# DrSleep/nas-segm-pytorch

Hardware: AMD Instinct MI355X
Metric: images/sec (fwd+bwd+optimizer step) WACV arch0 2048x1024 bs=4/GPU (higher is better)
Workload: dtype f32

## Files before the change

include/nasseg.h:

```cpp
#ifndef NASSEG_H
#define NASSEG_H

#include <stdint.h>

#ifdef __cplusplus
extern "C" {
#endif

const char* nasseg_last_error(void);
int nasseg_abi_version(void);
int nasseg_device_count(void);

int nasseg_dw_pack_weight(const float* w, float* wt, int C, int K, int flip, void* stream);
int nasseg_dwconv(const float* x, const float* wt, float* y, const float* in_scale,
                  const float* in_shift, int in_act, const float* scale, const float* shift, int act,
                  int B, int H, int W, int C, int Ho, int Wo, int K, int stride, int pad, int dil,
                  int transposed, float* stats, void* stream);
int nasseg_dwconv_strip_ok(int K, int stride, int dil);
int64_t nasseg_dwconv_stats_blocks(int B, int C, int Ho, int Wo, int K, int stride, int dil);
int nasseg_dwconv_bwd_data_bn(const float* dy, const float* wt, float* g, const float* z,
                              const float* scale, const float* shift, const float* mean,
                              const float* invstd, int act, int B, int H, int W, int C, int Ho,
                              int Wo, int K, int stride, int pad, int dil, int transposed,
                              float* stats, void* stream);
// ... 35 lines not shown
                    int in_act, const float* bn1_scale, const float* bn1_shift, const float* bn1_mean,
                    const float* bn1_invstd, int act1, const float* bn2_scale, const float* bn2_shift,
                    const float* bn2_mean, const float* bn2_invstd, const float* bn2_sums, int bn2_train, int bn2_act,
                    int B, int H, int W, int K, int C, int Ho, int Wo, int stride, float* stats, void* stream);

int nasseg_conv_pack_weight(const float* w, float* wp, int N, int K, int kh, int kw, int mode,
                            void* stream);
int nasseg_pack_weights(int count, const float* const* w, float* const* wp, const int* dims,
                        void* stream);
int nasseg_conv_fwd_pack_mode(int K, int kh, int kw);
int nasseg_conv_fwd(const float* x, int ldx, const float* wp, float* y, int ldy,
                    const float* in_scale, const float* in_shift, int in_act,
                    const float* out_scale, const float* out_shift, int out_act, const float* res,
                    int ldres, int B, int Hs, int Ws, int K, int Ho, int Wo, int N, int kh, int kw,
                    int stride, int pad, int dil, int transposed, float* stats, void* stream);
int64_t nasseg_conv_fwd_stats_blocks(int B, int Ho, int Wo, int N, int K, int pointwise);
int64_t nasseg_conv_fwd_stats_rows(int B, int Ho, int Wo, int N, int K, int kh, int kw, int stride, int pad, int dil);
int64_t nasseg_conv_pw_min_pixels(int64_t v);
int nasseg_conv_pwn_mode(int v);
int nasseg_conv_deep_k(int v);
int nasseg_pool_strip(int v);
int64_t nasseg_conv_pointwise_kernel(int B, int Ho, int Wo, int N, int K, int pointwise);
int64_t nasseg_conv_fwd_lds3x3(int B, int Ho, int Wo, int N, int K, int kh, int kw, int stride, int pad, int dil,
                               int with_stats);
int nasseg_conv_bwd_data_bn(const float* dy, int lddy, const float* wp, float* g, int ldg,
                            const float* z, int ldz, const float* scale, const float* shift,
                            const float* mean, const float* invstd, int act, int B, int Hs, int Ws,
                            int K, int Ho, int Wo, int N, int kh, int kw, int stride, int pad,
                            int dil, float* stats, void* stream);
int nasseg_conv_wgrad_lds3x3(int B, int Hs, int Ws, int K, int Ho, int Wo, int N, int kh, int kw, int stride,
// ... 16 lines not shown
int nasseg_dwconv_wgrad_bn(const float* x, const float* g, const float* z, float* dz, float* dw, float* ws,
                           const float* in_scale, const float* in_shift, int in_act, const float* bn_scale, const float* bn_shift,
                           const float* bn_mean, const float* bn_invstd, const float* bn_sums, int bn_train, int bn_act,
                           int B, int H, int W, int C, int Ho, int Wo, int K, int stride, int pad, int dil,
                           void* stream);
int64_t nasseg_conv_pw_bwd_slabs(int B, int H, int W, int K, int N);
int64_t nasseg_conv_pw_bwd_reads_z(int B, int H, int W, int K, int N);
int64_t nasseg_conv_pw_bwd_kernel_id(int B, int H, int W, int K, int N, int z_null);
int64_t nasseg_conv_pw_bwd_rz_min_pixels(int64_t v);
int nasseg_conv_pw_bwd_bn(const float* x, const float* g, const float* z, const float* wb, float* dx, float* dw,
                          float* ws, const float* in_scale, const float* in_shift, int in_act, int dx_act,
                          const float* bn_scale, const float* bn_shift, const float* bn_mean, const float* bn_invstd,
                          const float* bn_sums, int bn_train, int bn_act, int B, int H, int W, int K, int N,
                          const float* in_mean, const float* in_invstd, float* dx_stats, const float* dx_res,
                          void* stream);
int nasseg_conv_wgrad(const float* x, int ldx, const float* dy, int lddy, float* dw, float* ws,
                      const float* in_scale, const float* in_shift, int in_act, int B, int Hs,
                      int Ws, int K, int Ho, int Wo, int N, int kh, int kw, int stride, int pad,
                      int dil, void* stream);

int64_t nasseg_colred_workspace(int S, int64_t R, int C);
int nasseg_colred(int mode, const float* a, int64_t lda, const float* b, int64_t ldb,
                  const float* c, int64_t ldc, float* out, float* ws, int S, int64_t R, int C,
                  float mul, void* stream);
int nasseg_bn_stats(const float* x, int64_t ldx, int64_t M, int C, float eps, float momentum,
                    const float* gamma, const float* beta, float* mean, float* invstd,
                    float* scale, float* shift, float* running_mean, float* running_var,
                    int64_t* num_batches_tracked, float* ws, void* stream);
int nasseg_bn_finalize(float* partial, int nblk, int64_t M, int C, float eps, float momentum,
                       const float* gamma, const float* beta, float* mean, float* invstd,
// ... 294 lines not shown
                         const float* bn2_scale, const float* bn2_shift, const float* bn2_mean,
                         const float* bn2_invstd, const float* bn2_sums, int bn2_train, int bn2_act, int B, int H, int W,
                         int K, int C, int Ho, int Wo, int stride, float* stats, void* stream);
int nasseg_bf16_dwconv_bwd_bn(const nasseg_bf16_t* xz, const nasseg_bf16_t* g, const nasseg_bf16_t* z, const float* wt,
                              int wt_flipped, nasseg_bf16_t* ge, float* dw, float* ws, const float* in_scale, const float* in_shift,
                              const float* in_mean, const float* in_invstd, int in_act, const float* bn_scale,
                              const float* bn_shift, const float* bn_mean, const float* bn_invstd, const float* bn_sums,
                              int bn_train, int bn_act, int B, int H, int W, int C, int Ho, int Wo, int K, int stride,
                              int pad, int dil, float* stats, void* stream);
int nasseg_bf16_conv_pw_bwd_bn(const nasseg_bf16_t* x, const nasseg_bf16_t* g, const nasseg_bf16_t* z, const float* wb,
                               nasseg_bf16_t* dx, float* dw, float* ws, const float* in_scale, const float* in_shift,
                               int in_act, int dx_act, const float* bn_scale, const float* bn_shift, const float* bn_mean,
                               const float* bn_invstd, const float* bn_sums, int bn_train, int bn_act, int B, int H,
                               int W, int K, int N, const float* in_mean, const float* in_invstd, float* dx_stats,
                               const nasseg_bf16_t* dx_res, void* stream);
int nasseg_bf16_sepconv_fwd(const nasseg_bf16_t* x, const float* wdw, const float* wpw, nasseg_bf16_t* zdw,
                            nasseg_bf16_t* y, const float* in_scale, const float* in_shift, int in_act,
                            const float* out_scale, const float* out_shift, int out_act, int B, int H, int W, int C,
                            int Ho, int Wo, int N, int K, int stride, int pad, int dil, float* stats, void* stream);
int nasseg_bf16_affine_act(const nasseg_bf16_t* x, const float* scale, const float* shift, const nasseg_bf16_t* res,
                      nasseg_bf16_t* y, int64_t n, int C, int act, void* stream);
int nasseg_bf16_psum_bwd(const nasseg_bf16_t* dy, const nasseg_bf16_t* za, const float* tsa, int act_a, const float* ca,
                         nasseg_bf16_t* ga, float* part_a, const nasseg_bf16_t* zb, const float* tsb, int act_b,
                         const float* cb, nasseg_bf16_t* gb, float* part_b, float* cpart, int B, int H, int W, int C,
                         void* stream);
int nasseg_bf16_add_act2(const nasseg_bf16_t* xa, const float* sa, const float* ha, int act_a, const float* ca,
                         const nasseg_bf16_t* xb, const float* sb, const float* hb, int act_b, const float* cb,
                         nasseg_bf16_t* y, int64_t n, int C, void* stream);
int nasseg_bf16_bn_bwd_apply(const nasseg_bf16_t* dy, const nasseg_bf16_t* x, const float* scale, const float* shift,
                        const float* mean, const float* invstd, const float* sums, int64_t M,
// ... 178 lines not shown
                  int B, int H, int W, int C, int Ho, int Wo, int K, int stride, int pad, int dil,
                  int transposed, float* stats, void* stream);
int nasseg_bf16_dwconv_bwd_data_bn(const nasseg_bf16_t* dy, const float* wt, nasseg_bf16_t* g, const nasseg_bf16_t* z,
                              const float* scale, const float* shift, const float* mean,
                              const float* invstd, int act, int B, int H, int W, int C, int Ho,
                              int Wo, int K, int stride, int pad, int dil, int transposed,
                              float* stats, void* stream);
int nasseg_bf16_dwconv_wgrad(const nasseg_bf16_t* x, const nasseg_bf16_t* dy, float* dw, float* ws,
                        const float* in_scale, const float* in_shift, int in_act, int B, int H, int W,
                        int C, int Ho, int Wo, int K, int stride, int pad, int dil, void* stream);
int nasseg_bf16_conv_fwd(const nasseg_bf16_t* x, int ldx, const float* wp, nasseg_bf16_t* y, int ldy,
                    const float* in_scale, const float* in_shift, int in_act,
                    const float* out_scale, const float* out_shift, int out_act, const nasseg_bf16_t* res,
                    int ldres, int B, int Hs, int Ws, int K, int Ho, int Wo, int N, int kh, int kw,
                    int stride, int pad, int dil, int transposed, float* stats, void* stream);
int nasseg_bf16_conv_bwd_data_bn(const nasseg_bf16_t* dy, int lddy, const float* wp, nasseg_bf16_t* g, int ldg,
                            const nasseg_bf16_t* z, int ldz, const float* scale, const float* shift,
                            const float* mean, const float* invstd, int act, int B, int Hs, int Ws,
                            int K, int Ho, int Wo, int N, int kh, int kw, int stride, int pad,
                            int dil, float* stats, void* stream);
int nasseg_bf16_conv_wgrad_many(int count, const int64_t* desc, void* stream);
int nasseg_bf16_dwconv_wgrad_many(int count, const int64_t* desc, void* stream);
int nasseg_bf16_conv_wgrad_bn(const nasseg_bf16_t* x, int ldx, const nasseg_bf16_t* g, int ldg,
                              const nasseg_bf16_t* z, int ldz, nasseg_bf16_t* dz, int lddz, float* dw, float* ws,
                              const float* in_scale, const float* in_shift, int in_act, const float* bn_scale, const float* bn_shift,
                              const float* bn_mean, const float* bn_invstd, const float* bn_sums, int bn_train, int bn_act,
                              int B, int H, int W, int K, int N, void* stream);
int nasseg_bf16_conv_wgrad_bn_flat(const nasseg_bf16_t* x, int ldx, const nasseg_bf16_t* g, int ldg,
                                   const nasseg_bf16_t* z, int ldz, float* dw, float* ws, const float* bn_scale,
                                   const float* bn_shift, const float* bn_mean, const float* bn_invstd,
// ... 40 lines not shown
```

nas-segm-pytorch_amd/csrc/conv_fwd.hip:

```cpp
#include "conv_args.h"

#include <atomic>
#include <cstdio>
#include <cstdlib>

#if NASSEG_FP32_ONLY
std::atomic<int> g_conv_deep_k{1};
#else
extern std::atomic<int> g_conv_deep_k;
#endif

namespace {

enum { KM_VEC = 0, KM_SCALAR = 1, KM_FLAT = 2 };

#ifndef NASSEG_CONV_KU
#define NASSEG_CONV_KU 1
#endif
#ifndef NASSEG_PW_MIN_PIXELS
#define NASSEG_PW_MIN_PIXELS -2
#endif
#ifndef NASSEG_LDS3X3_VALU_TAIL
#define NASSEG_LDS3X3_VALU_TAIL 1
#endif
// ... 348 lines not shown
  p.nt = pw_round_tiles(cdiv(N, 16));
  if (!p.nt) return p;
  p.mt = p.nt <= 6 ? 2 : 1;
  const int KP = (K + 15) & ~15;
  p.lds = ((size_t)p.nt * 16 * (KP + 4) + 2 * KP + 4 * 2 * p.nt * 16) * sizeof(float);
  if (p.lds > (size_t)(64 << 10)) return p;
  int r = p.nt <= 2 ? 4 : (p.nt <= 4 ? 3 : (p.nt == 9 ? 3 : 2));
  const int by_lds = (int)((size_t)(160 << 10) / p.lds);
  if (r > by_lds) r = by_lds;
  const int64_t wg_tiles = cdiv64(cdiv64(M, 16 * p.mt), 4);
  p.grid = (int)(wg_tiles < 256LL * r ? wg_tiles : 256LL * r);
  p.ok = 1;
  return p;
}

template <int NT, int MT, int STATS>
__global__ __launch_bounds__(256) void conv_pw_kernel(FwdArgs a) {
  constexpr bool kSums = STATS == 1 || STATS == 2;
  constexpr int NPc = NT * 16;
  extern __shared__ float smem[];
  const int K = a.K, N = a.N;
  const int KP = (K + 15) & ~15, LSK = KP + 4, nkb = KP >> 4;
  float* wl = smem;
  float* psc = wl + NPc * LSK;
  float* psh = psc + KP;
  float* sred = psh + KP;
  const int tid = threadIdx.x;
  const int lane = tid & 63, wave = tid >> 6;
  const int j = lane & 15, kg = lane >> 4;
  const int Mtot = a.g.B * a.g.Ho * a.g.Wo;
  const int ntiles = (Mtot + 16 * MT - 1) / (16 * MT);

  for (int it = tid; it < NPc * (KP >> 2); it += 256) {
    const int n = it / (KP >> 2), k = (it - n * (KP >> 2)) * 4;
    const float4 v = keep_if(lda4(a.w + (int64_t)(n < N ? n : 0) * K + (k < K ? k : 0)), n < N && k < K);
    *reinterpret_cast<float4*>(&wl[n * LSK + k]) = v;
  }
  const bool pro = a.in_scale || a.in_shift || a.in_act;
  for (int k = tid; k < KP; k += 256) {
    psc[k] = (a.in_scale && k < K) ? a.in_scale[k] : 1.f;
    psh[k] = (a.in_shift && k < K) ? a.in_shift[k] : 0.f;
  }
  for (int t = tid; t < 4 * 2 * NPc; t += 256) sred[t] = 0.f;
  __syncthreads();
  const ActSel pact = act_sel(a.in_act);
  float* my_red = sred + wave * 2 * NPc;

  f32x4 acc[MT][NT];
#pragma unroll
  for (int mt = 0; mt < MT; ++mt)
#pragma unroll
    for (int nt = 0; nt < NT; ++nt) acc[mt][nt] = (f32x4){0.f, 0.f, 0.f, 0.f};

  const int wstride = gridDim.x * 4;
  int tl = blockIdx.x * 4 + wave, kl = 0;
  float4 ring[kPwD][MT];
  auto load_step = [&](float4* dst) {
    const int tc = tl < ntiles ? tl : ntiles - 1;
    const int k = kl * 16 + kg * 4;
#pragma unroll
    for (int mt = 0; mt < MT; ++mt) {
      const int m = tc * (16 * MT) + mt * 16 + j;
      dst[mt] = lda4(a.x + (int64_t)(m < Mtot ? m : Mtot - 1) * a.ldx + (k < K ? k : 0));
    }
    if (++kl == nkb) {
      kl = 0;
      tl += wstride;
    }
  };
#pragma unroll
  for (int d = 0; d < kPwD; ++d) load_step(ring[d]);

  int tc = blockIdx.x * 4 + wave, kc = 0;
  bool more = tc < ntiles;
  while (more) {
#pragma unroll
    for (int d = 0; d < kPwD; ++d) {
      if (tc >= ntiles) {
// ... 117 lines not shown
        for (int mt = 0; mt < MT; ++mt) acc[mt][nt] = (f32x4){0.f, 0.f, 0.f, 0.f};
        if ((nt & 1) == 1) __builtin_amdgcn_sched_barrier(0);
      }
    }
  }
  if (kSums) {
    __syncthreads();
    for (int t = tid; t < NPc; t += 256) {
      if (t < N) {
        float* po = a.stats + (int64_t)blockIdx.x * 2 * N + t;
        po[0] = (sred[t] + sred[2 * NPc + t]) + (sred[4 * NPc + t] + sred[6 * NPc + t]);
        po[N] = (sred[NPc + t] + sred[3 * NPc + t]) + (sred[5 * NPc + t] + sred[7 * NPc + t]);
      }
    }
  }
}

__global__ void conv_pack_kernel(const float* __restrict__ w, float* __restrict__ wp, int N, int K,
                                 int ntaps, int mode) {
  const int64_t i = (int64_t)blockIdx.x * blockDim.x + threadIdx.x;
  const int64_t total = (int64_t)ntaps * N * K;
  if (i >= total) return;
  int tap, n, k;
  if (mode == 0) {
    k = (int)(i % K);
    int64_t t = i / K;
    n = (int)(t % N);
    tap = (int)(t / N);
  } else if (mode == 1) {
    n = (int)(i % N);
// ... 565 lines not shown
  return NASSEG_OK;
}
int launch_pw(const FwdArgs& a, const PwFwdPlan& p, int stats, hipStream_t s) {
  switch (p.nt) {
    case 1: return launch_pw_nt<1, 2>(a, p, stats, s);
    case 2: return launch_pw_nt<2, 2>(a, p, stats, s);
    case 3: return launch_pw_nt<3, 2>(a, p, stats, s);
    case 4: return launch_pw_nt<4, 2>(a, p, stats, s);
    case 6: return launch_pw_nt<6, 2>(a, p, stats, s);
    case 9: return launch_pw_nt<9, 1>(a, p, stats, s);
    case 12: return launch_pw_nt<12, 1>(a, p, stats, s);
    default: return launch_pw_nt<14, 1>(a, p, stats, s);
  }
}

inline bool conv_small_ws(int64_t Mtot, int N, int K) {
  return g_conv_deep_k.load() != 0 && Mtot <= kDeepKMaxPixels && (N & 3) == 0 && (K & 3) == 0 && K >= 8 &&
         (int64_t)N * K <= 196608;
}

inline bool lds3x3_geometry(int B, int Ho, int Wo, int N, int K, int kh, int kw, int stride, int pad, int dil) {
  return kh == 3 && kw == 3 && stride == 1 && dil >= 1 && dil <= kLdsMaxDil && K * 9 > 64 && cdiv(N, 16) <= 4 &&
         Wo >= kLdsTW && Ho >= kLdsTH && B <= 65535 && pad >= 0 && pad <= 2 * dil;
}

inline int fwd_pack_mode(int K, int kh, int kw) { return (kh * kw > 1 && kh * kw * K <= 64) ? 2 : 0; }

int conv_dispatch(FwdArgs& a, int stats_mode, hipStream_t s) {
  const int K = a.K, N = a.N;
  const ConvGeom& g = a.g;
// ... 185 lines not shown
                    const float* in_scale, const float* in_shift, int in_act,
                    const float* out_scale, const float* out_shift, int out_act, const act_t* res,
                    int ldres, int B, int Hs, int Ws, int K, int Ho, int Wo, int N, int kh, int kw,
                    int stride, int pad, int dil, int transposed, float* stats, void* stream) {
  FwdArgs a = {};
  a.x = x; a.ldx = ldx; a.w = wp; a.y = y; a.ldy = ldy;
  a.in_scale = in_scale; a.in_shift = in_shift; a.in_act = in_act;
  a.out_scale = out_scale; a.out_shift = out_shift; a.out_act = out_act;
  a.res = res; a.ldres = ldres; a.stats = stats; a.K = K; a.N = N;
  a.g.B = B; a.g.Hs = Hs; a.g.Ws = Ws; a.g.Ho = Ho; a.g.Wo = Wo;
  a.g.kh = kh; a.g.kw = kw; a.g.stride = stride; a.g.pad = pad; a.g.dil = dil;
  a.g.transposed = transposed;
  return conv_dispatch(a, stats ? 1 : 0, (hipStream_t)stream);
}

int NASSEG_FN(conv_bwd_data_bn)(const act_t* dy, int lddy, const float* wp, act_t* g, int ldg,
                            const act_t* z, int ldz, const float* scale, const float* shift,
                            const float* mean, const float* invstd, int act, int B, int Hs, int Ws,
                            int K, int Ho, int Wo, int N, int kh, int kw, int stride, int pad,
                            int dil, float* stats, void* stream) {
  NASSEG_REQUIRE(z && (!stats || (scale && shift && mean && invstd)), "conv_bwd_data_bn: null argument");
  NASSEG_REQUIRE((ldz & 3) == 0 && ldz >= N, "conv_bwd_data_bn: bad ldz");
  FwdArgs a = {};
  a.x = dy; a.ldx = lddy; a.w = wp; a.y = g; a.ldy = ldg;
  a.stats = stats; a.K = K; a.N = N;
  a.bz = z; a.ldbz = ldz; a.b_scale = scale; a.b_shift = shift; a.b_mean = mean;
  a.b_invstd = invstd; a.b_act = act;
  a.g.B = B; a.g.Hs = Hs; a.g.Ws = Ws; a.g.Ho = Ho; a.g.Wo = Wo;
  a.g.kh = kh; a.g.kw = kw; a.g.stride = stride; a.g.pad = pad; a.g.dil = dil;
  a.g.transposed = 1;
// ... 5 lines not shown
```

nas-segm-pytorch_amd/csrc/conv_pwbwd.hip:

```cpp
#include <atomic>
#include <cstdlib>
#include <type_traits>

#include "conv_common.h"

#if NASSEG_FP32_ONLY
std::atomic<int64_t> g_pw_rz_min_pixels{1 << 18};
#else
extern std::atomic<int64_t> g_pw_rz_min_pixels;
#endif

namespace {

#ifndef NASSEG_PW_CHUNK
#define NASSEG_PW_CHUNK 3
#endif
#ifndef NASSEG_PW_RECOMPUTE_Z
#define NASSEG_PW_RECOMPUTE_Z 1
#endif
constexpr int kPwTile = 64;
constexpr int kPwMaxTiles = 24;

struct PwArgs {
  const act_t* x;
// ... 343 lines not shown
      __syncthreads();
      if (wave == 0) {
#pragma unroll
        for (int r = 0; r < 4; ++r) {
          const float v = acc2[nt][kt][r] + red[(0 * 64 + lane) * 4 + r] + red[(1 * 64 + lane) * 4 + r] +
                          red[(2 * 64 + lane) * 4 + r];
          const int n = nt * 16 + 4 * kg + r, k = kt * 16 + j;
          if (n < N && k < K) pout[(int64_t)n * K + k] = v;
        }
      }
    }
}

constexpr int kPwChunk = 64;
constexpr int kW2LS = kPwChunk + 4;
template <int KC, bool PRO>
__global__ __launch_bounds__(256, 2) void conv_pw_bwd_wide_kernel(PwArgs a) {
  extern __shared__ float smem[];
  constexpr int LS = kW2LS;
  float* dzt = smem;
  float* xt = dzt + kPwTile * LS;
  float* wt = xt + kPwTile * LS;
  float* wt0 = wt + kPwChunk * LS;
  float* ca = wt0 + kPwChunk * LS;
  float* cb = ca + 64;
  float* cd = cb + 64;
  float* cs = cd + 64;
  float* psc = cs + 64;
  float* psh = psc + KC * kPwChunk;
  const int tid = threadIdx.x;
  const int lane = tid & 63, wave = tid >> 6;
  const int j = lane & 15, kg = lane >> 4;
  const int N = a.N, K = a.K;
  for (int n = tid; n < 64; n += 256) {
    float va = 0.f, vb = 0.f, vd = 0.f, vs = 0.f;
    if (n < N) {
      const float sc = a.bn_scale[n];
      va = sc;
      vs = a.bn_act ? a.bn_shift[n] : 0.f;
      if (a.bn_train) {
        const float is = a.bn_invstd[n], mu = a.bn_mean[n];
        const float s0 = a.bn_sums[n] * a.invM, s1 = a.bn_sums[N + n] * a.invM;
        vb = -sc * is * s1;
        vd = sc * (mu * is * s1 - s0);
      }
    }
    ca[n] = va; cb[n] = vb; cd[n] = vd; cs[n] = vs;
  }
// ... 15 lines not shown
  const float m_lo = a.bn_act ? 0.f : -__builtin_inff();
  const float m_hi = a.bn_act == NASSEG_ACT_RELU6 ? 6.f : __builtin_inff();
  const int irow = tid >> 4, icol = (tid & 15) * 4;
  float4 XN[4], WN[4], GN[4], ZN[4];
  auto issue_gz = [&](int t0) {
#pragma unroll
    for (int u = 0; u < 4; ++u) {
      const int p = t0 + irow + 16 * u;
      const int64_t off = (int64_t)(p < p_end ? p : p_end - 1) * N + (icol < N ? icol : 0);
      GN[u] = lda4(a.g + off);
      ZN[u] = lda4(a.z + off);
    }
  };
  auto issue_xw = [&](int t0, int kc) {
    const int k = kc + icol;
#pragma unroll
    for (int u = 0; u < 4; ++u) {
      const int p = t0 + irow + 16 * u;
      XN[u] = lda4(a.x + (int64_t)(p < p_end ? p : p_end - 1) * K + (k < K ? k : 0));
      if (kc) {
        const int kw = kc + irow + 16 * u;
        WN[u] = ld4(a.wb + (int64_t)(kw < K ? kw : 0) * N + (icol < N ? icol : 0));
      }
    }
  };
  auto place_gz = [&](int t0) {
    const float4 va = ld4(ca + icol), vb = ld4(cb + icol), vd = ld4(cd + icol), vs = ld4(cs + icol);
#pragma unroll
    for (int u = 0; u < 4; ++u) {
      const int px = irow + 16 * u;
      const bool ok = t0 + px < p_end && icol < N;
      float4 gv = GN[u];
      const float4 zv = ZN[u];
      {
// ... 70 lines not shown
              const int n = ns * 16 + kg * 4;
              const float4 bv = *reinterpret_cast<const float4*>(brow + n);
              float4 av[NQ];
#pragma unroll
              for (int q = 0; q < NQ; ++q) av[q] = *reinterpret_cast<const float4*>(&wcur[(q * 16 + j) * LS + n]);
#pragma unroll
              for (int q = 0; q < NQ; ++q) acc1[q] = mfma16(av[q].x, bv.x, acc1[q]);
#pragma unroll
              for (int q = 0; q < NQ; ++q) acc1[q] = mfma16(av[q].y, bv.y, acc1[q]);
#pragma unroll
              for (int q = 0; q < NQ; ++q) acc1[q] = mfma16(av[q].z, bv.z, acc1[q]);
#pragma unroll
              for (int q = 0; q < NQ; ++q) acc1[q] = mfma16(av[q].w, bv.w, acc1[q]);
            }
            const bool pok = p < p_end;
            act_t* prow = a.dx + (int64_t)(pok ? p : p_begin) * K + kc + kg * 4;
#pragma unroll
            for (int q = 0; q < NQ; ++q) {
              const int kl = q * 16 + kg * 4;
              float4 o = make_float4(acc1[q][0], acc1[q][1], acc1[q][2], acc1[q][3]);
              if (a.dx_act)
                o = mul4(o, act_mask_of(*reinterpret_cast<const float4*>(&xt[(wave * 16 + j) * LS + kl]), a.dx_act));
              if (pok && kc + kl < K) sta4(prow + q * 16, a.dx_res ? add4(o, rres[q]) : o);
            }
          }
          if (own) {
            auto dw_chunk = [&](f32x4 (&acc)[4]) {
#pragma unroll 2
              for (int u = 0; u < kPwTile / 4; ++u) {
                const int pl = u * 4 + kg;
                const float av = dzt[pl * LS + wave * 16 + j];
// ... 21 lines not shown
      }
    }
  }
  if (own) {
    float* pout = a.partial + (int64_t)blockIdx.x * N * K;
#pragma unroll
    for (int c = 0; c < KC; ++c)
#pragma unroll
      for (int q = 0; q < 4; ++q)
#pragma unroll
        for (int r = 0; r < 4; ++r) {
          const int n = wave * 16 + 4 * kg + r, k = c * kPwChunk + q * 16 + j;
          if (n < N && k < K) pout[(int64_t)n * K + k] = acc2[c][q][r];
        }
  }
}

struct PwPlan {
  int ok, nt, kt, nslab, pix_per_slab, wide, rz;
};
inline int pw_round_nt(int nt) {
  const int allowed[] = {2, 3, 4, 6, 9, 12};
  for (int v : allowed)
    if (nt <= v) return v;
  return 0;
}
inline PwPlan pw_plan(int64_t M, int N, int K) {
  PwPlan p = {};
  if (N % 4 || K % 4 || N <= 0 || K <= 0 || M <= 0 || M >= 2147483647LL) return p;
  const int kt0 = cdiv(K, 16);
// ... 164 lines not shown
    PW_REBUILD(X)
#undef X
#define X(NT_, KT_) case pw_id(NT_, KT_, 0): pw_launch<NT_, KT_>(a, p.nslab, pro, s); break;
    PW_NARROW(X)
#undef X
    default: return nasseg_fail(NASSEG_ERR_UNSUPPORTED, "conv_pw_bwd_bn: no kernel with id %d", id);
  }
  NASSEG_LAUNCH_CHECK("conv_pw_bwd_kernel");
  if (!dw) return NASSEG_OK;
  const float* parts[1] = {ws};
  float* outs[1] = {dw};
  const int dims[5] = {p.nslab, 1, N, K, 0};
  return nasseg_wgrad_finalize_many(1, parts, outs, dims, stream);
}

}
```

nas-segm-pytorch_amd/functional.py:

```python
import collections
import ctypes
import os
import weakref

import numpy as np
import torch

from ._lib import LaunchProfiler, NassegError, current_stream, lib, ptr, require_device

ACT_NONE, ACT_RELU, ACT_RELU6 = 0, 1, 2
RED_SUM, RED_SUMSQ, RED_DOT2, RED_DOT1 = 0, 1, 3, 4


_BF16_PREFIX = "nasseg_bf16_"


def _k(name, t):
    if t.dtype == torch.float32:
        return name
    return _BF16_PREFIX + name[7:]


def _to_dtype(t, dtype):
    if t.dtype == dtype:
# ... 1469 lines not shown
                lib.call(_k("nasseg_chan_copy", dy), ptr(dy), Ct, off, ptr(dx), C, 0, None, 0, 0,
                         B * Ho * Wo, C, ACT_NONE, ACT_NONE, s)
            else:
                nws = lib.query("nasseg_bilinear_bwd_workspace", B, H, W, C, Ho, Wo)
                lib.call(_k("nasseg_bilinear_bwd", dy), ptr(dy), Ct, off, ptr(dx), B, H, W, C, Ho, Wo,
                         ptr(_ws(dy, nws)) if nws else None, s)
            grads.append(dx)
            off += C
        return (None, None, None) + tuple(grads)


def concat_resize(tensors, size, relu=False):
    return _ConcatResize.apply(int(size[0]), int(size[1]), ACT_RELU if relu else ACT_NONE, *tensors)


def _bn_relu_pw_forward(x, scale, shift, wp, N, res=None):
    B, C, H, W = x.shape
    out = _new(x, B, N, H, W)
    lib.call(_k("nasseg_conv_fwd", x), ptr(x), C, ptr(wp), ptr(out), N, ptr(scale), ptr(shift), ACT_RELU, None, None,
             ACT_NONE, ptr(res), N if res is not None else 0, B, H, W, C, H, W, N, 1, 1, 1, 0, 1, 0, None,
             current_stream())
    return out


def _bn_relu_pw_backward(dout, x, parts, wb):
    mean, invstd, scale, shift = parts
    B, C, H, W = x.shape
    N = dout.shape[1]
    s = current_stream()
    nb = lib.query("nasseg_conv_fwd_stats_blocks", B, H, W, C, N, 2)
# ... 1700 lines not shown
```

nas-segm-pytorch_amd/nn/micro_decoders.py:

```python
import torch.nn as nn

from .. import functional as F
from ..rl.genotypes import AGG_OP_NAMES, OP_NAMES, OP_NAMES_WACV
from .layer_factory import AGG_OPS, OPS, conv3x3, conv_bn_relu, run_op
from .modules import TREE_VERSION, FusedSequential


def _takes_pending_types():
    from .layer_factory import DilConv, SepConv

    return (SepConv, DilConv, FusedSequential)


_TAKES_PENDING = _takes_pending_types()


def _applies_pending(op):
    from .layer_factory import SepConv
    from .modules import _chainable, _flatten

    if isinstance(op, SepConv):
        return True
    if isinstance(op, FusedSequential):
        mods = _flatten(op._modules.values())
# ... 23 lines not shown
        if not queue:
            raise F.NassegError("node {} has more consumers than the decoder counted ({})".format(idx, len(flags)))
        return queue.pop(0)

    def check_all_taken(self):
        left = dict((idx, len(q)) for idx, q in self.out.items() if q)
        if left:
            raise F.NassegError("decoder nodes fanned out to consumers that never came: {}".format(left))


def _hw(t):
    return (int(t.size(2)), int(t.size(3)))


def collect_all(feats, collect_indices, relu=False):
    first = feats[collect_indices[0]]
    cur = _hw(first)
    pieces = [[first, []]]
    for i in collect_indices[1:]:
        t = feats[i]
        size = _hw(t)
        if cur[0] > size[0]:
            pieces.append([t, [cur]])
        elif size[0] > cur[0]:
            for piece in pieces:
                piece[1].append(size)
            cur = size
            pieces.append([t, []])
        else:
            if size[1] != cur[1]:
                raise RuntimeError("Sizes of tensors must match except in dimension 1")
            pieces.append([t, []])
    if len(pieces) == 1 and not relu:
        return first
    ready = []
    for t, chain in pieces:
        for hop in chain[:-1]:
            t = F.bilinear_resize(t, hop)
        ready.append(t)
    return F.concat_resize(ready, cur, relu=relu)


def _sum_to_larger(x1, x2):
    s1, s2 = _hw(x1), _hw(x2)
    if s1 > s2:
        x2 = F.bilinear_resize(F.materialize(x2), s1)
    elif s1 < s2:
        x1 = F.bilinear_resize(F.materialize(x1), s2)
    return F.add(x1, x2)


def _param_header(n_params):
    return "#PARAMS\n\n {:3.2f}M".format(n_params / 1e6)


# ... 150 lines not shown
        maps = [getattr(self, "adapt{}".format(n + 1))(t) for n, t in enumerate(x)]
        uses = [[] for _ in range(len(maps) + len(self.conns))]
        for block, (a, b) in enumerate(self.conns):
            uses[a].append(False)
            uses[b].append(False)
            uses[len(x) + block].append(False)
        for i in self.collect_inds:
            uses[i].append(False)
        handles = _Handles(maps, uses)
        aux_outs = []
        for block, (cell, head, (a, b)) in enumerate(zip(self.cells, self.aux_clfs, self.conns)):
            maps.append(cell(handles.take(a), handles.take(b)))
            aux_outs.append(head(handles.take(len(x) + block)))
        picked = {i: handles.take(i) for i in self.collect_inds}
        handles.check_all_taken()
        out = collect_all(picked, self.collect_inds)
        return self.conv_clf(self.pre_clf(out, relu_in=True)), aux_outs


class TemplateDecoder(nn.Module):

    def __init__(self, inp_sizes, num_classes, config, agg_size=64, num_pools=4, repeats=1,
                 stride_power=1, **kwargs):
        super(TemplateDecoder, self).__init__()
        widths = list(inp_sizes)
        n_scales = len(widths)
        templates, structure = config
        n_blocks = len(structure)
        widths += [0] * n_blocks
        self.agg_size = agg_size
        self._ops = nn.ModuleList()
        self._pos = []
# ... 74 lines not shown
                reps.append((left, right, out_id))
                left, right = right, out_id
            plan.append(reps)
        for i in self._collect_inds:
            uses[i].append(False)
        values = maps + [None] * (len(uses) - len(maps))
        handles = _Handles(values, uses)
        for reps, ops in zip(plan, self._ops):
            for rep, (left, right, out_id) in enumerate(reps):
                defer = getattr(ops[rep * 3 + 2], "accepts_pending", False)
                a = run_op(ops[rep * 3], handles.take(left), defer)
                b = run_op(ops[rep * 3 + 1], handles.take(right), defer)
                values[out_id] = ops[rep * 3 + 2](a, b)
        picked = {i: handles.take(i) for i in self._collect_inds}
        handles.check_all_taken()
        out = collect_all(picked, self._collect_inds)
        return self.conv_clf(self.pre_clf(out, relu_in=True))
```

Before: 309.3.

## Fuse decoder concat into pre-classifier pointwise conv via segmented inputs

Adds segmented-input variants of the pointwise conv forward and wide backward kernels. Each K-chunk is resolved to a pointer and leading dimension in one of up to eight source tensors through a small table in shared memory. The decoder's collect step then feeds the pieces straight into the pre_clf 1x1 conv+BN+ReLU. This skips materialising the concatenated tensor and, in backward, the split of its gradient. The cost is extra LDS, a per-load indirection, and eligibility checks that fall back to the old path.

```diff
diff --git a/include/nasseg.h b/include/nasseg.h
--- a/include/nasseg.h
+++ b/include/nasseg.h
@@ -73,6 +73,11 @@
                     const float* out_scale, const float* out_shift, int out_act, const float* res,
                     int ldres, int B, int Hs, int Ws, int K, int Ho, int Wo, int N, int kh, int kw,
                     int stride, int pad, int dil, int transposed, float* stats, void* stream);
+int nasseg_conv_pw_cat_fwd(const float* x0, const float* x1, const float* x2, const float* x3, const float* x4,
+                           const float* x5, const float* x6, const float* x7, int c0, int c1, int c2, int c3, int c4,
+                           int c5, int c6, int c7, int nseg, const float* wp, float* y, int ldy, const float* in_scale,
+                           const float* in_shift, int in_act, const float* out_scale, const float* out_shift,
+                           int out_act, int B, int H, int W, int N, float* stats, void* stream);
 int64_t nasseg_conv_fwd_stats_blocks(int B, int Ho, int Wo, int N, int K, int pointwise);
 int64_t nasseg_conv_fwd_stats_rows(int B, int Ho, int Wo, int N, int K, int kh, int kw, int stride, int pad, int dil);
 int64_t nasseg_conv_pw_min_pixels(int64_t v);
@@ -119,6 +124,14 @@
                           const float* bn_sums, int bn_train, int bn_act, int B, int H, int W, int K, int N,
                           const float* in_mean, const float* in_invstd, float* dx_stats, const float* dx_res,
                           void* stream);
+int nasseg_conv_pw_cat_bwd_bn(const float* x0, const float* x1, const float* x2, const float* x3, const float* x4,
+                              const float* x5, const float* x6, const float* x7, float* dx0, float* dx1, float* dx2,
+                              float* dx3, float* dx4, float* dx5, float* dx6, float* dx7, int c0, int c1, int c2,
+                              int c3, int c4, int c5, int c6, int c7, int nseg, const float* g, const float* z,
+                              const float* wb, float* dw, float* ws, const float* in_scale, const float* in_shift,
+                              int in_act, int dx_act, const float* bn_scale, const float* bn_shift,
+                              const float* bn_mean, const float* bn_invstd, const float* bn_sums, int bn_train,
+                              int bn_act, int B, int H, int W, int N, void* stream);
 int nasseg_conv_wgrad(const float* x, int ldx, const float* dy, int lddy, float* dw, float* ws,
                       const float* in_scale, const float* in_shift, int in_act, int B, int Hs,
                       int Ws, int K, int Ho, int Wo, int N, int kh, int kw, int stride, int pad,
@@ -443,6 +456,17 @@
                                const float* bn_invstd, const float* bn_sums, int bn_train, int bn_act, int B, int H,
                                int W, int K, int N, const float* in_mean, const float* in_invstd, float* dx_stats,
                                const nasseg_bf16_t* dx_res, void* stream);
+int nasseg_bf16_conv_pw_cat_bwd_bn(const nasseg_bf16_t* x0, const nasseg_bf16_t* x1, const nasseg_bf16_t* x2,
+                                   const nasseg_bf16_t* x3, const nasseg_bf16_t* x4, const nasseg_bf16_t* x5,
+                                   const nasseg_bf16_t* x6, const nasseg_bf16_t* x7, nasseg_bf16_t* dx0,
+                                   nasseg_bf16_t* dx1, nasseg_bf16_t* dx2, nasseg_bf16_t* dx3, nasseg_bf16_t* dx4,
+                                   nasseg_bf16_t* dx5, nasseg_bf16_t* dx6, nasseg_bf16_t* dx7, int c0, int c1, int c2,
+                                   int c3, int c4, int c5, int c6, int c7, int nseg, const nasseg_bf16_t* g,
+                                   const nasseg_bf16_t* z, const float* wb, float* dw, float* ws,
+                                   const float* in_scale, const float* in_shift, int in_act, int dx_act,
+                                   const float* bn_scale, const float* bn_shift, const float* bn_mean,
+                                   const float* bn_invstd, const float* bn_sums, int bn_train, int bn_act, int B, int H,
+                                   int W, int N, void* stream);
 int nasseg_bf16_sepconv_fwd(const nasseg_bf16_t* x, const float* wdw, const float* wpw, nasseg_bf16_t* zdw,
                             nasseg_bf16_t* y, const float* in_scale, const float* in_shift, int in_act,
                             const float* out_scale, const float* out_shift, int out_act, int B, int H, int W, int C,
@@ -651,6 +675,13 @@
                     const float* out_scale, const float* out_shift, int out_act, const nasseg_bf16_t* res,
                     int ldres, int B, int Hs, int Ws, int K, int Ho, int Wo, int N, int kh, int kw,
                     int stride, int pad, int dil, int transposed, float* stats, void* stream);
+int nasseg_bf16_conv_pw_cat_fwd(const nasseg_bf16_t* x0, const nasseg_bf16_t* x1, const nasseg_bf16_t* x2,
+                                const nasseg_bf16_t* x3, const nasseg_bf16_t* x4, const nasseg_bf16_t* x5,
+                                const nasseg_bf16_t* x6, const nasseg_bf16_t* x7, int c0, int c1, int c2, int c3,
+                                int c4, int c5, int c6, int c7, int nseg, const float* wp, nasseg_bf16_t* y, int ldy,
+                                const float* in_scale, const float* in_shift, int in_act, const float* out_scale,
+                                const float* out_shift, int out_act, int B, int H, int W, int N, float* stats,
+                                void* stream);
 int nasseg_bf16_conv_bwd_data_bn(const nasseg_bf16_t* dy, int lddy, const float* wp, nasseg_bf16_t* g, int ldg,
                             const nasseg_bf16_t* z, int ldz, const float* scale, const float* shift,
                             const float* mean, const float* invstd, int act, int B, int Hs, int Ws,
diff --git a/nas-segm-pytorch_amd/csrc/conv_fwd.hip b/nas-segm-pytorch_amd/csrc/conv_fwd.hip
--- a/nas-segm-pytorch_amd/csrc/conv_fwd.hip
+++ b/nas-segm-pytorch_amd/csrc/conv_fwd.hip
@@ -386,8 +386,15 @@
   return p;
 }
 
-template <int NT, int MT, int STATS>
-__global__ __launch_bounds__(256) void conv_pw_kernel(FwdArgs a) {
+constexpr int kCatMax = 8;
+struct CatSegs {
+  const act_t* x[kCatMax];
+  int c[kCatMax];
+  int n;
+};
+
+template <int NT, int MT, int STATS, bool SEG>
+__device__ __forceinline__ void conv_pw_body(const FwdArgs& a, const CatSegs* sg) {
   constexpr bool kSums = STATS == 1 || STATS == 2;
   constexpr int NPc = NT * 16;
   extern __shared__ float smem[];
@@ -414,6 +421,25 @@
     psh[k] = (a.in_shift && k < K) ? a.in_shift[k] : 0.f;
   }
   for (int t = tid; t < 4 * 2 * NPc; t += 256) sred[t] = 0.f;
+  const act_t** segp = reinterpret_cast<const act_t**>(sred + 4 * 2 * NPc);
+  int* segld = reinterpret_cast<int*>(segp + nkb);
+  if (SEG) {
+    for (int kb = tid; kb < nkb; kb += 256) {
+      const int k = kb * 16;
+      const act_t* p = sg->x[0];
+      int ld = sg->c[0], k0 = 0, end = sg->c[0];
+#pragma unroll
+      for (int i = 1; i < kCatMax; ++i) {
+        const bool in = i < sg->n && k >= end;
+        p = in ? sg->x[i] : p;
+        ld = in ? sg->c[i] : ld;
+        k0 = in ? end : k0;
+        end += i < sg->n ? sg->c[i] : 0;
+      }
+      segp[kb] = p + (k - k0);
+      segld[kb] = ld;
+    }
+  }
   __syncthreads();
   const ActSel pact = act_sel(a.in_act);
   float* my_red = sred + wave * 2 * NPc;
@@ -430,10 +456,12 @@
   auto load_step = [&](float4* dst) {
     const int tc = tl < ntiles ? tl : ntiles - 1;
     const int k = kl * 16 + kg * 4;
+    const act_t* xb = SEG ? segp[kl] + kg * 4 : a.x + (k < K ? k : 0);
+    const int ldx = SEG ? segld[kl] : a.ldx;
 #pragma unroll
     for (int mt = 0; mt < MT; ++mt) {
       const int m = tc * (16 * MT) + mt * 16 + j;
-      dst[mt] = lda4(a.x + (int64_t)(m < Mtot ? m : Mtot - 1) * a.ldx + (k < K ? k : 0));
+      dst[mt] = lda4(xb + (int64_t)(m < Mtot ? m : Mtot - 1) * ldx);
     }
     if (++kl == nkb) {
       kl = 0;
@@ -581,6 +609,15 @@
       }
     }
   }
+}
+
+template <int NT, int MT, int STATS>
+__global__ __launch_bounds__(256) void conv_pw_kernel(FwdArgs a) {
+  conv_pw_body<NT, MT, STATS, false>(a, nullptr);
+}
+template <int NT, int MT, int STATS>
+__global__ __launch_bounds__(256) void conv_pw_cat_kernel(FwdArgs a, CatSegs sg) {
+  conv_pw_body<NT, MT, STATS, true>(a, &sg);
 }
 
 __global__ void conv_pack_kernel(const float* __restrict__ w, float* __restrict__ wp, int N, int K,
@@ -1176,6 +1213,15 @@
   }
 }
 
+template <int NT>
+int launch_pw_cat_nt(const FwdArgs& a, const CatSegs& sg, const PwFwdPlan& p, size_t lds, int stats, hipStream_t s) {
+  const dim3 grid(p.grid), block(256);
+  if (stats) hipLaunchKernelGGL((conv_pw_cat_kernel<NT, 2, 1>), grid, block, lds, s, a, sg);
+  else hipLaunchKernelGGL((conv_pw_cat_kernel<NT, 2, 0>), grid, block, lds, s, a, sg);
+  NASSEG_LAUNCH_CHECK("conv_pw_cat_kernel");
+  return NASSEG_OK;
+}
+
 inline bool conv_small_ws(int64_t Mtot, int N, int K) {
   return g_conv_deep_k.load() != 0 && Mtot <= kDeepKMaxPixels && (N & 3) == 0 && (K & 3) == 0 && K >= 8 &&
          (int64_t)N * K <= 196608;
@@ -1391,6 +1437,51 @@
   return conv_dispatch(a, stats ? 1 : 0, (hipStream_t)stream);
 }
 
+int NASSEG_FN(conv_pw_cat_fwd)(const act_t* x0, const act_t* x1, const act_t* x2, const act_t* x3, const act_t* x4,
+                               const act_t* x5, const act_t* x6, const act_t* x7, int c0, int c1, int c2, int c3,
+                               int c4, int c5, int c6, int c7, int nseg, const float* wp, act_t* y, int ldy,
+                               const float* in_scale, const float* in_shift, int in_act, const float* out_scale,
+                               const float* out_shift, int out_act, int B, int H, int W, int N, float* stats,
+                               void* stream) {
+  NASSEG_REQUIRE(nseg >= 1 && nseg <= kCatMax && wp && y, "conv_pw_cat_fwd: bad arguments");
+  NASSEG_REQUIRE(B > 0 && H > 0 && W > 0 && (int64_t)B * H * W < 2147483647LL, "conv_pw_cat_fwd: bad geometry");
+  const act_t* xs[kCatMax] = {x0, x1, x2, x3, x4, x5, x6, x7};
+  const int cs[kCatMax] = {c0, c1, c2, c3, c4, c5, c6, c7};
+  CatSegs sg = {};
+  sg.n = nseg;
+  int K = 0;
+  for (int i = 0; i < nseg; ++i) {
+    NASSEG_REQUIRE(xs[i] && cs[i] > 0 && cs[i] % 16 == 0, "conv_pw_cat_fwd: segment %d is null or not a multiple of 16 wide", i);
+    sg.x[i] = xs[i];
+    sg.c[i] = cs[i];
+    K += cs[i];
+  }
+  NASSEG_REQUIRE(N > 0 && N <= 64 && (N & 3) == 0 && (ldy & 3) == 0 && ldy >= N, "conv_pw_cat_fwd: bad N=%d ldy=%d", N, ldy);
+  NASSEG_REQUIRE(!stats || !(out_scale || out_shift || out_act), "conv_pw_cat_fwd: statistics need no output epilogue");
+  const int64_t M = (int64_t)B * H * W;
+  const PwFwdPlan p = pw_fwd_plan(M, N, K, 1);
+  if (nasseg_internal_pwn_plan(M, N, K, 1).ok || !p.ok || p.nt > 4)
+    return nasseg_fail(NASSEG_ERR_UNSUPPORTED, "conv_pw_cat_fwd: K=%d N=%d over %lld pixels is not a conv_pw_kernel call",
+                       K, N, (long long)M);
+  const size_t lds = p.lds + (size_t)(K >> 4) * (sizeof(void*) + sizeof(int));
+  NASSEG_REQUIRE(lds <= (size_t)(64 << 10) && (size_t)(160 << 10) / lds == (size_t)(160 << 10) / p.lds,
+                 "conv_pw_cat_fwd: no room for the segment table");
+  FwdArgs a = {};
+  a.w = wp; a.y = y; a.ldy = ldy;
+  a.in_scale = in_scale; a.in_shift = in_shift; a.in_act = in_act;
+  a.out_scale = out_scale; a.out_shift = out_shift; a.out_act = out_act;
+  a.stats = stats; a.K = K; a.N = N;
+  a.g.B = B; a.g.Hs = H; a.g.Ws = W; a.g.Ho = H; a.g.Wo = W;
+  a.g.kh = 1; a.g.kw = 1; a.g.stride = 1;
+  hipStream_t s = (hipStream_t)stream;
+  switch (p.nt) {
+    case 1: return launch_pw_cat_nt<1>(a, sg, p, lds, stats ? 1 : 0, s);
+    case 2: return launch_pw_cat_nt<2>(a, sg, p, lds, stats ? 1 : 0, s);
+    case 3: return launch_pw_cat_nt<3>(a, sg, p, lds, stats ? 1 : 0, s);
+    default: return launch_pw_cat_nt<4>(a, sg, p, lds, stats ? 1 : 0, s);
+  }
+}
+
 int NASSEG_FN(conv_bwd_data_bn)(const act_t* dy, int lddy, const float* wp, act_t* g, int ldg,
                             const act_t* z, int ldz, const float* scale, const float* shift,
                             const float* mean, const float* invstd, int act, int B, int Hs, int Ws,
diff --git a/nas-segm-pytorch_amd/csrc/conv_pwbwd.hip b/nas-segm-pytorch_amd/csrc/conv_pwbwd.hip
--- a/nas-segm-pytorch_amd/csrc/conv_pwbwd.hip
+++ b/nas-segm-pytorch_amd/csrc/conv_pwbwd.hip
@@ -381,8 +381,15 @@
 
 constexpr int kPwChunk = 64;
 constexpr int kW2LS = kPwChunk + 4;
-template <int KC, bool PRO>
-__global__ __launch_bounds__(256, 2) void conv_pw_bwd_wide_kernel(PwArgs a) {
+constexpr int kCatMax = 8;
+struct CatSegsBwd {
+  const act_t* x[kCatMax];
+  act_t* dx[kCatMax];
+  int c[kCatMax];
+  int n;
+};
+template <int KC, bool PRO, bool SEG>
+__device__ __forceinline__ void conv_pw_bwd_wide_body(const PwArgs& a, const CatSegsBwd* sg) {
   extern __shared__ float smem[];
   constexpr int LS = kW2LS;
   float* dzt = smem;
@@ -395,10 +402,35 @@
   float* cs = cd + 64;
   float* psc = cs + 64;
   float* psh = psc + KC * kPwChunk;
+  const act_t** chx = reinterpret_cast<const act_t**>(psh + KC * kPwChunk);
+  act_t** chdx = reinterpret_cast<act_t**>(psh + KC * kPwChunk) + KC;
+  int* chld = reinterpret_cast<int*>(chdx + KC);
   const int tid = threadIdx.x;
   const int lane = tid & 63, wave = tid >> 6;
   const int j = lane & 15, kg = lane >> 4;
   const int N = a.N, K = a.K;
+  if (SEG) {
+    if (tid < KC) {
+      const int k = tid * kPwChunk;
+      const act_t* p = sg->x[0];
+      act_t* d = sg->dx[0];
+      int ld = sg->c[0], k0 = 0, end = sg->c[0];
+#pragma unroll
+      for (int i = 1; i < kCatMax; ++i) {
+        const bool in = i < sg->n && k >= end;
+        p = in ? sg->x[i] : p;
+        d = in ? sg->dx[i] : d;
+        ld = in ? sg->c[i] : ld;
+        k0 = in ? end : k0;
+        end += i < sg->n ? sg->c[i] : 0;
+      }
+      const int off = k < K ? k - k0 : 0;
+      chx[tid] = p + off;
+      chdx[tid] = d + off;
+      chld[tid] = ld;
+    }
+    __syncthreads();
+  }
   for (int n = tid; n < 64; n += 256) {
     float va = 0.f, vb = 0.f, vd = 0.f, vs = 0.f;
     if (n < N) {
@@ -444,10 +476,12 @@
   };
   auto issue_xw = [&](int t0, int kc) {
     const int k = kc + icol;
+    const act_t* xb = SEG ? chx[kc / kPwChunk] + (k < K ? icol : 0) : a.x + (k < K ? k : 0);
+    const int ldx = SEG ? chld[kc / kPwChunk] : K;
 #pragma unroll
     for (int u = 0; u < 4; ++u) {
       const int p = t0 + irow + 16 * u;
-      XN[u] = lda4(a.x + (int64_t)(p < p_end ? p : p_end - 1) * K + (k < K ? k : 0));
+      XN[u] = lda4(xb + (int64_t)(p < p_end ? p : p_end - 1) * ldx);
       if (kc) {
         const int kw = kc + irow + 16 * u;
         WN[u] = ld4(a.wb + (int64_t)(kw < K ? kw : 0) * N + (icol < N ? icol : 0));
@@ -548,7 +582,8 @@
               for (int q = 0; q < NQ; ++q) acc1[q] = mfma16(av[q].w, bv.w, acc1[q]);
             }
             const bool pok = p < p_end;
-            act_t* prow = a.dx + (int64_t)(pok ? p : p_begin) * K + kc + kg * 4;
+            act_t* prow = SEG ? chdx[c] + (int64_t)(pok ? p : p_begin) * chld[c] + kg * 4
+                              : a.dx + (int64_t)(pok ? p : p_begin) * K + kc + kg * 4;
 #pragma unroll
             for (int q = 0; q < NQ; ++q) {
               const int kl = q * 16 + kg * 4;
@@ -600,6 +635,14 @@
           if (n < N && k < K) pout[(int64_t)n * K + k] = acc2[c][q][r];
         }
   }
+}
+template <int KC, bool PRO>
+__global__ __launch_bounds__(256, 2) void conv_pw_bwd_wide_kernel(PwArgs a) {
+  conv_pw_bwd_wide_body<KC, PRO, false>(a, nullptr);
+}
+template <int KC, bool PRO>
+__global__ __launch_bounds__(256, 2) void conv_pw_bwd_wide_cat_kernel(PwArgs a, CatSegsBwd sg) {
+  conv_pw_bwd_wide_body<KC, PRO, true>(a, &sg);
 }
 
 struct PwPlan {
@@ -794,4 +837,79 @@
   return nasseg_wgrad_finalize_many(1, parts, outs, dims, stream);
 }
 
-}
+int NASSEG_FN(conv_pw_cat_bwd_bn)(const act_t* x0, const act_t* x1, const act_t* x2, const act_t* x3,
+                                  const act_t* x4, const act_t* x5, const act_t* x6, const act_t* x7, act_t* dx0,
+                                  act_t* dx1, act_t* dx2, act_t* dx3, act_t* dx4, act_t* dx5, act_t* dx6, act_t* dx7,
+                                  int c0, int c1, int c2, int c3, int c4, int c5, int c6, int c7, int nseg,
+                                  const act_t* g, const act_t* z, const float* wb, float* dw, float* ws,
+                                  const float* in_scale, const float* in_shift, int in_act, int dx_act,
+                                  const float* bn_scale, const float* bn_shift, const float* bn_mean,
+                                  const float* bn_invstd, const float* bn_sums, int bn_train, int bn_act, int B, int H,
+                                  int W, int N, void* stream) {
+  NASSEG_REQUIRE(nseg >= 1 && nseg <= kCatMax && g && z && wb && ws && bn_scale, "conv_pw_cat_bwd_bn: null tensor");
+  NASSEG_REQUIRE((!bn_train || (bn_mean && bn_invstd && bn_sums)) && (!bn_act || bn_shift),
+                 "conv_pw_cat_bwd_bn: missing BatchNorm tensors");
+  NASSEG_REQUIRE(B > 0 && H > 0 && W > 0, "conv_pw_cat_bwd_bn: bad geometry");
+  NASSEG_REQUIRE(!dx_act || dx_act == in_act,
+                 "conv_pw_cat_bwd_bn: dx can only be masked with the derivative of the input activation");
+  const act_t* xs[kCatMax] = {x0, x1, x2, x3, x4, x5, x6, x7};
+  act_t* dxs[kCatMax] = {dx0, dx1, dx2, dx3, dx4, dx5, dx6, dx7};
+  const int cs[kCatMax] = {c0, c1, c2, c3, c4, c5, c6, c7};
+  CatSegsBwd sg = {};
+  sg.n = nseg;
+  int K = 0;
+  for (int i = 0; i < nseg; ++i) {
+    NASSEG_REQUIRE(xs[i] && dxs[i] && cs[i] > 0 && cs[i] % 16 == 0,
+                   "conv_pw_cat_bwd_bn: segment %d is null or not a multiple of 16 wide", i);
+    NASSEG_REQUIRE(K % kPwChunk == 0, "conv_pw_cat_bwd_bn: segment %d does not start on a 64-channel chunk", i);
+    sg.x[i] = xs[i];
+    sg.dx[i] = dxs[i];
+    sg.c[i] = cs[i];
+    K += cs[i];
+  }
+  const int64_t M = (int64_t)B * H * W;
+  const PwPlan p = pw_plan(M, N, K);
+  const int id = pw_kernel_id(p, false);
+  if (!p.ok || !p.wide || id < 0)
+    return nasseg_fail(NASSEG_ERR_UNSUPPORTED, "conv_pw_cat_bwd_bn: K=%d N=%d is not a wide-kernel call", K, N);
+  PwArgs a = {};
+  a.g = g; a.z = z; a.partial = ws; a.wb = wb;
+  a.in_scale = in_scale; a.in_shift = in_shift; a.in_act = in_act;
+  a.bn_scale = bn_scale; a.bn_shift = bn_shift; a.bn_mean = bn_mean; a.bn_invstd = bn_invstd;
+  a.bn_sums = bn_sums; a.bn_train = bn_train; a.bn_act = bn_act;
+  a.invM = (float)(1.0 / (double)M);
+  a.dx_act = dx_act;
+  a.K = K; a.N = N; a.KP = (K + 15) & ~15; a.NP = (N + 15) & ~15;
+  a.M = (int)M; a.pix_per_slab = p.pix_per_slab;
+  const bool pro = in_scale || in_shift || in_act;
+  hipStream_t s = (hipStream_t)stream;
+  const int kc_n = id - kPwIdWide;
+  const size_t ldsw2 = ((size_t)4 * kPwTile * kW2LS + 4 * 64 + 2 * p.kt * kPwChunk) * sizeof(float) +
+                       (size_t)kc_n * (2 * sizeof(void*) + sizeof(int));
+#define PW_WIDE_CAT(KC_)                                                                                             \
+  do {                                                                                                               \
+    if (ldsw2 > (64 << 10)) {          \
+      (void)hipFuncSetAttribute((const void*)conv_pw_bwd_wide_cat_kernel<KC_, true>,                                 \
+                                hipFuncAttributeMaxDynamicSharedMemorySize, (int)ldsw2);                             \
+      (void)hipFuncSetAttribute((const void*)conv_pw_bwd_wide_cat_kernel<KC_, false>,                                \
+                                hipFuncAttributeMaxDynamicSharedMemorySize, (int)ldsw2);                             \
+    }                                                                                                                \
+    if (pro) hipLaunchKernelGGL((conv_pw_bwd_wide_cat_kernel<KC_, true>), dim3(p.nslab), dim3(256), ldsw2, s, a, sg); \
+    else hipLaunchKernelGGL((conv_pw_bwd_wide_cat_kernel<KC_, false>), dim3(p.nslab), dim3(256), ldsw2, s, a, sg);    \
+  } while (0)
+  switch (kc_n) {
+    case 2: PW_WIDE_CAT(2); break;
+    case 3: PW_WIDE_CAT(3); break;
+    case 4: PW_WIDE_CAT(4); break;
+    default: return nasseg_fail(NASSEG_ERR_UNSUPPORTED, "conv_pw_cat_bwd_bn: no kernel with id %d", id);
+  }
+#undef PW_WIDE_CAT
+  NASSEG_LAUNCH_CHECK("conv_pw_bwd_wide_cat_kernel");
+  if (!dw) return NASSEG_OK;
+  const float* parts_w[1] = {ws};
+  float* outs_w[1] = {dw};
+  const int dims_w[5] = {p.nslab, 1, N, K, 0};
+  return nasseg_wgrad_finalize_many(1, parts_w, outs_w, dims_w, stream);
+}
+
+}
diff --git a/nas-segm-pytorch_amd/functional.py b/nas-segm-pytorch_amd/functional.py
--- a/nas-segm-pytorch_amd/functional.py
+++ b/nas-segm-pytorch_amd/functional.py
@@ -1507,6 +1507,132 @@
     return _ConcatResize.apply(int(size[0]), int(size[1]), ACT_RELU if relu else ACT_NONE, *tensors)
 
 
+COLLECT_DIRECT = os.environ.get("NASSEG_COLLECT_DIRECT", "1") != "0"
+_COLLECT_MAX = 8
+
+
+def collect_conv_ok(widths, B, H, W, N, itemsize, with_grad):
+    K = sum(widths)
+    if not (COLLECT_DIRECT and 2 <= len(widths) <= _COLLECT_MAX):
+        return False
+    if any(c <= 0 or c % 16 for c in widths) or any(c % 64 for c in widths[:-1]):
+        return False
+    if K > 384 or N > 64 or N % 4:
+        return False
+    if lib.query("nasseg_conv_pointwise_kernel", B, H, W, N, K, 1) != 1:
+        return False
+    if with_grad:
+        if not (FUSE_PW_BWD and _PW_BWD_WIDE and K > 64 and B * H * W >= _PW_BWD_WIDE_MIN_PIXELS):
+            return False
+        if B * H * W * (K + N) * itemsize <= _PW_BWD_MIN_BYTES:
+            return False
+        if not 10000 <= lib.query("nasseg_conv_pw_bwd_kernel_id", B, H, W, K, N, 0) <= 10004:
+            return False
+    return True
+
+
+def _seg_args(tensors, widths):
+    pad = _COLLECT_MAX - len(tensors)
+    return [ptr(t) for t in tensors] + [None] * pad, list(widths) + [0] * pad
+
+
+class _CollectConv(torch.autograd.Function):
+
+    @staticmethod
+    def forward(ctx, cfg, weight, gamma, beta, rm, rv, nbt, *xs):
+        Ho, Wo, in_act, act, grad_mode, training, momentum, eps = cfg
+        xs = [_cl(x) for x in xs]
+        B = xs[0].shape[0]
+        s = current_stream()
+        segs, shapes = [], []
+        for x in xs:
+            _, C, H, W = x.shape
+            if x.shape[0] != B:
+                raise NassegError("collect_conv: batch sizes differ")
+            if (H, W) != (Ho, Wo):
+                y = _new(x, B, C, Ho, Wo)
+                lib.call(_k("nasseg_bilinear_fwd", x), ptr(x), ptr(y), C, 0, B, H, W, C, Ho, Wo, ACT_NONE, s)
+                x = y
+            segs.append(x)
+            shapes.append((C, H, W))
+        widths = [c for c, _, _ in shapes]
+        N, K, M = weight.shape[0], sum(widths), B * Ho * Wo
+        if tuple(weight.shape) != (N, K, 1, 1):
+            raise NassegError("collect_conv: weight {} does not match {} collected channels".format(
+                tuple(weight.shape), K))
+        needs_grad = grad_mode and any(ctx.needs_input_grad)
+        w = weight.contiguous()
+        packed = _pack_many(segs[0], [(w, "fwd")] + ([(w, 1)] if needs_grad else []))
+        z = _new(segs[0], B, N, Ho, Wo)
+        fold = not training and not needs_grad
+        bn = (gamma, beta, rm, rv, nbt)
+        stats, parts = _bn_alloc(z, N, training, M, z.shape)
+        scale, shift = parts[2:]
+        part, nblk = None, 0
+        if not training:
+            _bn_fill(parts, N, M, bn, False, momentum, eps)
+        else:
+            nblk = lib.query("nasseg_conv_fwd_stats_rows", B, Ho, Wo, N, K, 1, 1, 1, 0, 1)
+            part = _rows_ws(z, nblk, N)
+        o_sc, o_sh, o_act = (scale, shift, act) if fold else (None, None, ACT_NONE)
+        pts, cs = _seg_args(segs, widths)
+        lib.call(_k("nasseg_conv_pw_cat_fwd", z), *(pts + cs + [len(segs), ptr(packed[0]), ptr(z), N, None, None,
+                 in_act, ptr(o_sc), ptr(o_sh), o_act, B, Ho, Wo, N, ptr(part), s]))
+        if fold:
+            return z
+        if training:
+            _bn_fill(parts, N, M, bn, True, momentum, eps, z, (part, nblk))
+        y = _affine_act(z, scale, shift, None, act)
+        if needs_grad:
+            ctx.save_for_backward(z, stats, w, packed[1], *segs)
+            ctx.cfg = (cfg, shapes)
+        return y
+
+    @staticmethod
+    def backward(ctx, dy):
+        (Ho, Wo, in_act, act, _, training, _, _), shapes = ctx.cfg
+        z, stats, w, wb = ctx.saved_tensors[:4]
+        segs = ctx.saved_tensors[4:]
+        need = ctx.needs_input_grad
+        g = _cl(dy)
+        B, N = z.shape[0], z.shape[1]
+        widths = [c for c, _, _ in shapes]
+        K, M = sum(widths), B * Ho * Wo
+        s = current_stream()
+        mean, invstd, scale, shift = _bn_parts(stats, N)
+        sums = _vec(g, 2 * N)
+        _bn_bwd_reduce(g, z, scale, shift, mean, invstd, act, sums, M, N, False)
+        dwt = torch.empty_like(w)
+        nsl = lib.query("nasseg_conv_pw_bwd_slabs", B, Ho, Wo, K, N)
+        ws = _ws(z, nsl * N * K)
+        dsegs = [_new(g, B, c, Ho, Wo) for c in widths]
+        pts, cs = _seg_args(segs, widths)
+        dpts, _ = _seg_args(dsegs, widths)
+        lib.call(_k("nasseg_conv_pw_cat_bwd_bn", z), *(pts + dpts + cs + [len(segs), ptr(g), ptr(z), ptr(wb),
+                 _finish_wgrad(ws, dwt, 1, N, K, 0), ptr(ws), None, None, in_act, in_act, ptr(scale), ptr(shift),
+                 ptr(mean), ptr(invstd), ptr(sums), int(training), act, B, Ho, Wo, N, s]))
+        grads = []
+        for i, ((C, H, W), d) in enumerate(zip(shapes, dsegs)):
+            if not need[7 + i]:
+                d = None
+            elif (H, W) != (Ho, Wo):
+                dx = _new(d, B, C, H, W)
+                nws = lib.query("nasseg_bilinear_bwd_workspace", B, H, W, C, Ho, Wo)
+                lib.call(_k("nasseg_bilinear_bwd", d), ptr(d), C, 0, ptr(dx), B, H, W, C, Ho, Wo,
+                         ptr(_ws(d, nws)) if nws else None, s)
+                d = dx
+            grads.append(d)
+        return (None, dwt if need[1] else None, sums[N:2 * N] if need[2] else None, sums[0:N] if need[3] else None,
+                None, None, None) + tuple(grads)
+
+
+def collect_conv(pieces, size, weight, gamma, beta, running_mean, running_var, num_batches_tracked, training,
+                 momentum, eps, act=ACT_RELU, relu_in=True):
+    cfg = (int(size[0]), int(size[1]), ACT_RELU if relu_in else ACT_NONE, int(act), torch.is_grad_enabled(), bool(training), float(momentum), float(eps))
+    return _CollectConv.apply(cfg, weight, gamma, beta, running_mean, running_var,
+                              num_batches_tracked if training else None, *pieces)
+
+
 def _bn_relu_pw_forward(x, scale, shift, wp, N, res=None):
     B, C, H, W = x.shape
     out = _new(x, B, N, H, W)
diff --git a/nas-segm-pytorch_amd/nn/micro_decoders.py b/nas-segm-pytorch_amd/nn/micro_decoders.py
--- a/nas-segm-pytorch_amd/nn/micro_decoders.py
+++ b/nas-segm-pytorch_amd/nn/micro_decoders.py
@@ -1,9 +1,10 @@
+import torch
 import torch.nn as nn
 
 from .. import functional as F
 from ..rl.genotypes import AGG_OP_NAMES, OP_NAMES, OP_NAMES_WACV
 from .layer_factory import AGG_OPS, OPS, conv3x3, conv_bn_relu, run_op
-from .modules import TREE_VERSION, FusedSequential
+from .modules import TREE_VERSION, FusedSequential, _bn_fusable, _chainable
 
 
 def _takes_pending_types():
@@ -61,6 +62,13 @@
 
 
 def collect_all(feats, collect_indices, relu=False):
+    ready, cur = _collect_pieces(feats, collect_indices)
+    if len(ready) == 1 and not relu:
+        return ready[0]
+    return F.concat_resize(ready, cur, relu=relu)
+
+
+def _collect_pieces(feats, collect_indices):
     first = feats[collect_indices[0]]
     cur = _hw(first)
     pieces = [[first, []]]
@@ -78,14 +86,35 @@
             if size[1] != cur[1]:
                 raise RuntimeError("Sizes of tensors must match except in dimension 1")
             pieces.append([t, []])
-    if len(pieces) == 1 and not relu:
-        return first
     ready = []
     for t, chain in pieces:
         for hop in chain[:-1]:
             t = F.bilinear_resize(t, hop)
         ready.append(t)
-    return F.concat_resize(ready, cur, relu=relu)
+    return ready, cur
+
+
+def collect_pre_clf(decoder, feats, collect_indices):
+    ready, cur = _collect_pieces(feats, collect_indices)
+    mods = list(decoder.pre_clf._modules.values()) if isinstance(decoder.pre_clf, FusedSequential) else []
+    direct = (len(mods) == 3 and _chainable(mods[0]) and not mods[0].is_depthwise and _bn_fusable(mods[1])
+              and isinstance(mods[2], nn.ReLU) and not isinstance(mods[2], nn.ReLU6)
+              and mods[0].kernel_size == (1, 1) and mods[0].stride == (1, 1) and mods[0].padding == (0, 0)
+              and all(isinstance(t, torch.Tensor) and t.dim() == 4 and t.dtype == ready[0].dtype for t in ready))
+    if direct:
+        conv, bn = mods[0], mods[1]
+        pieces_grad = any(t.requires_grad for t in ready)
+        with_grad = torch.is_grad_enabled() and (pieces_grad or conv.weight.requires_grad or bn.weight.requires_grad
+                                                 or bn.bias.requires_grad)
+        direct = ((not with_grad or (pieces_grad and conv.weight.requires_grad))
+                  and sum(t.shape[1] for t in ready) == conv.in_channels
+                  and F.collect_conv_ok([int(t.shape[1]) for t in ready], int(ready[0].shape[0]), cur[0], cur[1],
+                                        conv.out_channels, ready[0].element_size(), with_grad))
+    if direct:
+        return F.collect_conv(ready, cur, conv.weight, bn.weight, bn.bias, bn.running_mean, bn.running_var,
+                              bn.num_batches_tracked, bn.training, bn.momentum, bn.eps, F.ACT_RELU)
+    out = ready[0] if len(ready) == 1 else F.concat_resize(ready, cur)
+    return decoder.pre_clf(out, relu_in=True)
 
 
 def _sum_to_larger(x1, x2):
@@ -266,8 +295,7 @@
             aux_outs.append(head(handles.take(len(x) + block)))
         picked = {i: handles.take(i) for i in self.collect_inds}
         handles.check_all_taken()
-        out = collect_all(picked, self.collect_inds)
-        return self.conv_clf(self.pre_clf(out, relu_in=True)), aux_outs
+        return self.conv_clf(collect_pre_clf(self, picked, self.collect_inds)), aux_outs
 
 
 class TemplateDecoder(nn.Module):
@@ -372,5 +400,4 @@
                 values[out_id] = ops[rep * 3 + 2](a, b)
         picked = {i: handles.take(i) for i in self._collect_inds}
         handles.check_all_taken()
-        out = collect_all(picked, self._collect_inds)
-        return self.conv_clf(self.pre_clf(out, relu_in=True))
+        return self.conv_clf(collect_pre_clf(self, picked, self._collect_inds))
```

New measurement: 311.9, median of 6. Within noise of the previous version (+0.8%).
